# SajayR/TRIAD

Measured on AMD Instinct MI355X. Metric: tri-modal triples/sec (whole node) + loss parity, B=256 at 1/2/4/8 MI355X, higher is better.
Workload: dtype bf16

## Files before the change

### triad_amd/csrc/gemm.hip

```cpp
#include "common.h"

namespace {

constexpr int BM = 128, BN = 128, BK = 64;
constexpr int A_ELEMS = BM * BK, B_ELEMS = BK * BN;

__device__ __forceinline__ int kc_off(int m, int chunk) { return m * BK + ((chunk ^ ((m >> 1) & 7)) << 3); }
__device__ __forceinline__ int nc_off(int k, int col) {
  return k * BN + ((((col >> 3) ^ ((k & 3) << 2))) << 3) + (col & 7);
}

template <bool A_KCONTIG>
__device__ __forceinline__ void stage_a_piece(const bf16* __restrict__ A, long long lda, int m0, int k0, bf16* dst,
                                              int wave, int lane, int u) {
  const int inst = wave * 4 + u;
  if (A_KCONTIG) {
    const int m = inst * 8 + (lane >> 3), cp = lane & 7;
    const int c = cp ^ ((m >> 1) & 7);
    glds16(A + (size_t)(m0 + m) * lda + k0 + c * 8, dst + inst * 512);
  } else {
    const int k = inst * 4 + (lane >> 4), cp = lane & 15;
    const int c = cp ^ ((k & 3) << 2);
    glds16(A + (size_t)(k0 + k) * lda + m0 + c * 8, dst + inst * 512);
  }
}

template <bool A_KCONTIG>
__device__ __forceinline__ void stage_a(const bf16* __restrict__ A, long long lda, int m0, int k0, bf16* dst,
                                        int wave, int lane) {
#pragma unroll
  for (int u = 0; u < 4; ++u) stage_a_piece<A_KCONTIG>(A, lda, m0, k0, dst, wave, lane, u);
}


template <bool B_KCONTIG>
__device__ __forceinline__ void stage_b(const bf16* __restrict__ B, long long ldb, int n0, int k0, bf16* dst,
                                        int wave, int lane) {
  stage_a<B_KCONTIG>(B, ldb, n0, k0, dst, wave, lane);
}

__device__ __forceinline__ bf16x8 frag_tr(const bf16* img, int n0, int s, int lane) {
  const int g = lane >> 4, i = lane & 15, q = i >> 2, p = i & 3, hh = g >> 1;
  const int col = n0 + 16 * (g & 1) + 4 * p;
  const int k0 = 16 * s + 8 * hh + q;
  const s16x4 lo = lds_tr16(img + nc_off(k0, col));
  const s16x4 hi = lds_tr16(img + nc_off(k0 + 4, col));
  bf16x8 r;
  s16x4* rp = (s16x4*)&r;
  rp[0] = lo;
  rp[1] = hi;
  return r;
}

__device__ __forceinline__ float bias_at(const void* bias, int bias_bf16, int n) {
  if (!bias) return 0.f;
  return bias_bf16 ? (float)((const bf16*)bias)[n] : ((const float*)bias)[n];
}

__device__ __forceinline__ void tile_split(int xsplit, int& tile, int& split) {
  const int T = gridDim.x;
  if (xsplit) {
    const int L = blockIdx.y * T + blockIdx.x, c = L % 8, i = L / 8;
    tile = i % T;
    split = c + 8 * (i / T);
    return;
  }
  const int bid = blockIdx.x, q8 = T / 8, r8 = T % 8, x = bid % 8;
  tile = (x < r8 ? x * (q8 + 1) : r8 * (q8 + 1) + (x - r8) * q8) + bid / 8;
  split = blockIdx.y;
}

template <bool A_KCONTIG, bool B_KCONTIG, typename OutT>
__global__ __launch_bounds__(256, 2) void gemm_kernel(const bf16* __restrict__ A, long long lda,
                                                      const bf16* __restrict__ B, long long ldb,
                                                      int M, int N, int Kd, const float* __restrict__ alpha_p,
                                                      OutT* __restrict__ C, long long ldc, int k_per_split,
                                                      long long slab_stride, const void* __restrict__ bias, int bias_bf16, int xsplit) {
  __shared__ __attribute__((aligned(16))) bf16 lds[2 * (A_ELEMS + B_ELEMS)];
  const int lane = threadIdx.x & 63, wave = __builtin_amdgcn_readfirstlane(threadIdx.x >> 6);
  const int wm = wave >> 1, wn = wave & 1;
  const int h = lane >> 5;

  int swz, split;
  tile_split(xsplit, swz, split);
  const int ntn = N / BN;
  const int m0 = (swz / ntn) * BM, n0 = (swz % ntn) * BN;

  f32x16 acc[2][2];
#pragma unroll
  for (int a = 0; a < 2; ++a)
#pragma unroll
    for (int b = 0; b < 2; ++b) acc[a][b] = (f32x16){};

  const int kbeg = split * k_per_split;
  const int nk = min(k_per_split, Kd - kbeg) / BK;
  C += (size_t)split * slab_stride;
  if (nk > 0) {
    stage_a<A_KCONTIG>(A, lda, m0, kbeg, lds, wave, lane);
    stage_b<B_KCONTIG>(B, ldb, n0, kbeg, lds + A_ELEMS, wave, lane);
  }
  for (int kt = 0; kt < nk; ++kt) {
    lds_dma_barrier();
    bf16* const nb = lds + ((kt + 1) & 1) * (A_ELEMS + B_ELEMS);
    const bool pf = kt + 1 < nk;
    if (pf) {
      stage_a<A_KCONTIG>(A, lda, m0, kbeg + (kt + 1) * BK, nb, wave, lane);
      stage_b<B_KCONTIG>(B, ldb, n0, kbeg + (kt + 1) * BK, nb + A_ELEMS, wave, lane);
    }
    const bf16* ai = lds + (kt & 1) * (A_ELEMS + B_ELEMS);
    const bf16* bi = ai + A_ELEMS;
#pragma unroll
    for (int s = 0; s < BK / 16; ++s) {
      bf16x8 af[2], bfr[2];
#pragma unroll
      for (int t = 0; t < 2; ++t) {
        const int mrow = wm * 64 + t * 32;
        if (A_KCONTIG) {
          af[t] = *(const bf16x8*)(ai + kc_off(mrow + (lane & 31), 2 * s + h));
        } else {
          af[t] = frag_tr(ai, mrow, s, lane);
        }
        const int ncol = wn * 64 + t * 32;
        if (B_KCONTIG) {
          bfr[t] = *(const bf16x8*)(bi + kc_off(ncol + (lane & 31), 2 * s + h));
        } else {
          bfr[t] = frag_tr(bi, ncol, s, lane);
        }
      }
#pragma unroll
      for (int a = 0; a < 2; ++a)
#pragma unroll
        for (int b = 0; b < 2; ++b) {
          acc[a][b] = mfma32(af[a], bfr[b], acc[a][b]);
        }
    }
  }

  const float alpha = alpha_p ? *alpha_p : 1.f;
#pragma unroll
  for (int a = 0; a < 2; ++a)
#pragma unroll
    for (int b = 0; b < 2; ++b) {
      const int n = n0 + wn * 64 + b * 32 + (lane & 31);
      const float bn = bias_at(bias, bias_bf16, n);
#pragma unroll
      for (int v = 0; v < 16; ++v) {
        const int m = m0 + wm * 64 + a * 32 + (v & 3) + 8 * (v >> 2) + 4 * h;
        C[(size_t)m * ldc + n] = (OutT)(alpha * acc[a][b][v] + bn);
      }
    }
}

constexpr int GB_M = 256, GB_NB = 3;
constexpr int GB_A = GB_M * BK, GB_ST = GB_A + B_ELEMS;
constexpr int GB_PIECES = 6;


template <bool A_KCONTIG, bool B_KCONTIG>
__device__ __forceinline__ void gb_piece(const bf16* __restrict__ A, long long lda, const bf16* __restrict__ B,
                                         long long ldb, int m0, int n0, int k0, bf16* dst, int wave, int lane,
                                         int u) {
  if (u < 4) {
    const int inst = wave * 4 + u;
    if (A_KCONTIG) {
      const int m = inst * 8 + (lane >> 3), cp = lane & 7;
      const int c = cp ^ ((m >> 1) & 7);
      glds16(A + (size_t)(m0 + m) * lda + k0 + c * 8, dst + inst * 512);
    } else {
      const int half = inst >> 4, ii = inst & 15;
      const int k = ii * 4 + (lane >> 4), cp = lane & 15;
      const int c = cp ^ ((k & 3) << 2);
      glds16(A + (size_t)(k0 + k) * lda + m0 + half * 128 + c * 8, dst + half * (BK * 128) + ii * 512);
    }
  } else {
    const int inst = wave * 2 + (u - 4);
    bf16* bd = dst + GB_A;
    if (B_KCONTIG) {
      const int n = inst * 8 + (lane >> 3), cp = lane & 7;
      const int c = cp ^ ((n >> 1) & 7);
      glds16(B + (size_t)(n0 + n) * ldb + k0 + c * 8, bd + inst * 512);
    } else {
      const int k = inst * 4 + (lane >> 4), cp = lane & 15;
      const int c = cp ^ ((k & 3) << 2);
      glds16(B + (size_t)(k0 + k) * ldb + n0 + c * 8, bd + inst * 512);
    }
  }
}

template <bool A_KCONTIG, bool B_KCONTIG, typename OutT>
__global__ __launch_bounds__(512, 1) void gemm_big_kernel(const bf16* __restrict__ A, long long lda,
                                                          const bf16* __restrict__ B, long long ldb, int M, int N,
                                                          int Kd, const float* __restrict__ alpha_p,
                                                          OutT* __restrict__ C, long long ldc, int k_per_split,
                                                          long long slab_stride, const void* __restrict__ bias, int bias_bf16, int xsplit) {
  __shared__ __attribute__((aligned(16))) bf16 lds[GB_NB * GB_ST];
  const int lane = threadIdx.x & 63, wave = __builtin_amdgcn_readfirstlane(threadIdx.x >> 6);
  const int wm = wave >> 1, wn = wave & 1;
  const int h = lane >> 5;
  int swz, split;
  tile_split(xsplit, swz, split);
  const int ntn = N / BN;
  const int m0 = (swz / ntn) * GB_M, n0 = (swz % ntn) * BN;

  f32x16 acc[2][2];
#pragma unroll
  for (int a = 0; a < 2; ++a)
#pragma unroll
    for (int b = 0; b < 2; ++b) acc[a][b] = (f32x16){};

  const int kbeg = split * k_per_split;
  const int nk = __builtin_amdgcn_readfirstlane(max(0, min(k_per_split, Kd - kbeg)) / BK);
  C += (size_t)split * slab_stride;
#pragma unroll
  for (int p = 0; p < GB_NB - 1; ++p)
    if (p < nk)
#pragma unroll
      for (int u = 0; u < GB_PIECES; ++u)
        gb_piece<A_KCONTIG, B_KCONTIG>(A, lda, B, ldb, m0, n0, kbeg + p * BK, lds + p * GB_ST, wave, lane, u);
  for (int kt = 0; kt < nk; ++kt) {
    if (kt + 1 < nk) TRIAD_VMCNT(GB_PIECES);
    else asm volatile("s_waitcnt vmcnt(0)" ::: "memory");
    __syncthreads();
    const bool pf = kt + GB_NB - 1 < nk;
    bf16* const nb = lds + ((kt + GB_NB - 1) % GB_NB) * GB_ST;
    const int kn = kbeg + (kt + GB_NB - 1) * BK;
    const bf16* ai = lds + (kt % GB_NB) * GB_ST;
    const bf16* bi = ai + GB_A;
#pragma unroll
    for (int s = 0; s < BK / 16; ++s) {
      bf16x8 af[2], bfr[2];
#pragma unroll
      for (int t = 0; t < 2; ++t) {
        const int mrow = wm * 64 + t * 32;
        if (A_KCONTIG) af[t] = *(const bf16x8*)(ai + kc_off(mrow + (lane & 31), 2 * s + h));
        else af[t] = frag_tr(ai + (mrow >> 7) * (BK * 128), mrow & 127, s, lane);
        const int ncol = wn * 64 + t * 32;
        if (B_KCONTIG) bfr[t] = *(const bf16x8*)(bi + kc_off(ncol + (lane & 31), 2 * s + h));
        else bfr[t] = frag_tr(bi, ncol, s, lane);
      }
#pragma unroll
      for (int a = 0; a < 2; ++a)
#pragma unroll
        for (int b = 0; b < 2; ++b) {
          acc[a][b] = mfma32(af[a], bfr[b], acc[a][b]);
          const int mi = s * 4 + a * 2 + b;
          if ((mi & 1) && mi / 2 < GB_PIECES) {
            __builtin_amdgcn_sched_barrier(0);
            if (pf) gb_piece<A_KCONTIG, B_KCONTIG>(A, lda, B, ldb, m0, n0, kn, nb, wave, lane, mi / 2);
            __builtin_amdgcn_sched_barrier(0);
          }
        }
    }
  }

  const float alpha = alpha_p ? *alpha_p : 1.f;
#pragma unroll
  for (int a = 0; a < 2; ++a)
#pragma unroll
    for (int b = 0; b < 2; ++b) {
      const int n = n0 + wn * 64 + b * 32 + (lane & 31);
      const float bn = bias_at(bias, bias_bf16, n);
#pragma unroll
      for (int v = 0; v < 16; ++v) {
        const int m = m0 + wm * 64 + a * 32 + (v & 3) + 8 * (v >> 2) + 4 * h;
        C[(size_t)m * ldc + n] = (OutT)(alpha * acc[a][b][v] + bn);
      }
    }
}

constexpr int GW_M = 256, GW_N = 256;
constexpr int GW_A = GW_M * BK, GW_ST = GW_A + GW_N * BK;

template <bool KCONTIG>
__device__ __forceinline__ void gw_piece_one(const bf16* __restrict__ X, long long ld, int r0, int k0, bf16* img,
                                             int inst, int lane) {
  if (KCONTIG) {
    const int m = inst * 8 + (lane >> 3), cp = lane & 7;
    const int c = cp ^ ((m >> 1) & 7);
    glds16(X + (size_t)(r0 + m) * ld + k0 + c * 8, img + inst * 512);
  } else {
    const int half = inst >> 4, ii = inst & 15;
    const int k = ii * 4 + (lane >> 4), cp = lane & 15;
    const int c = cp ^ ((k & 3) << 2);
    glds16(X + (size_t)(k0 + k) * ld + r0 + half * 128 + c * 8, img + half * (BK * 128) + ii * 512);
  }
}

template <bool KCONTIG>
__device__ __forceinline__ bf16x8 gw_frag(const bf16* img, int row, int s, int lane) {
  if (KCONTIG) return *(const bf16x8*)(img + kc_off(row + (lane & 31), 2 * s + (lane >> 5)));
  return frag_tr(img + (row >> 7) * (BK * 128), row & 127, s, lane);
}

constexpr int GE_PIECES = 8;

template <bool A_KCONTIG, bool B_KCONTIG>
__device__ __forceinline__ void ge_piece(const bf16* __restrict__ A, long long lda, const bf16* __restrict__ B,
                                         long long ldb, int m0, int n0, int k0, bf16* dst, int wave, int lane,
                                         int u) {
  if (u < 4) gw_piece_one<A_KCONTIG>(A, lda, m0, k0, dst, wave * 4 + u, lane);
  else gw_piece_one<B_KCONTIG>(B, ldb, n0, k0, dst + GW_A, wave * 4 + (u - 4), lane);
}

template <bool A_KCONTIG, bool B_KCONTIG, typename OutT>
__global__ __launch_bounds__(512, 1) void gemm_w8_kernel(const bf16* __restrict__ A, long long lda,
                                                         const bf16* __restrict__ B, long long ldb, int M, int N,
                                                         int Kd, const float* __restrict__ alpha_p,
                                                         OutT* __restrict__ C, long long ldc, int k_per_split,
                                                         long long slab_stride, const void* __restrict__ bias, int bias_bf16, int xsplit) {
  __shared__ __attribute__((aligned(16))) bf16 lds[2 * GW_ST];
  const int lane = threadIdx.x & 63, wave = __builtin_amdgcn_readfirstlane(threadIdx.x >> 6);
  const int wm = wave >> 2, wn = wave & 3;
  const int h = lane >> 5;
  int swz, split;
  tile_split(xsplit, swz, split);
  const int ntn = N / GW_N;
  const int m0 = (swz / ntn) * GW_M, n0 = (swz % ntn) * GW_N;

  f32x16 acc[4][2];
#pragma unroll
  for (int a = 0; a < 4; ++a)
#pragma unroll
    for (int b = 0; b < 2; ++b) acc[a][b] = (f32x16){};

  const int kbeg = split * k_per_split;
  const int nk = __builtin_amdgcn_readfirstlane(max(0, min(k_per_split, Kd - kbeg)) / BK);
  C += (size_t)split * slab_stride;
  if (nk > 0)
#pragma unroll
    for (int u = 0; u < GE_PIECES; ++u)
      ge_piece<A_KCONTIG, B_KCONTIG>(A, lda, B, ldb, m0, n0, kbeg, lds, wave, lane, u);
  for (int kt = 0; kt < nk; ++kt) {
    asm volatile("s_waitcnt vmcnt(0)" ::: "memory");
    __syncthreads();
    const bool pf = kt + 1 < nk;
    bf16* const nb = lds + ((kt + 1) & 1) * GW_ST;
    const int kn = kbeg + (kt + 1) * BK;
    const bf16* ai = lds + (kt & 1) * GW_ST;
    const bf16* bi = ai + GW_A;
    bf16x8 af[2][4], bfr[2][2];
#pragma unroll
    for (int t = 0; t < 4; ++t) af[0][t] = gw_frag<A_KCONTIG>(ai, wm * 128 + t * 32, 0, lane);
#pragma unroll
    for (int t = 0; t < 2; ++t) bfr[0][t] = gw_frag<B_KCONTIG>(bi, wn * 64 + t * 32, 0, lane);
#pragma unroll
    for (int s = 0; s < BK / 16; ++s) {
      const int cur = s & 1;
#pragma unroll
      for (int a = 0; a < 4; ++a)
#pragma unroll
        for (int b = 0; b < 2; ++b) {
          acc[a][b] = mfma32(af[cur][a], bfr[cur][b], acc[a][b]);
          const int j = a * 2 + b, mi = s * 8 + j;
          if (s + 1 < BK / 16 && j < 6) {
            __builtin_amdgcn_sched_barrier(0);
            if (j < 4) af[cur ^ 1][j] = gw_frag<A_KCONTIG>(ai, wm * 128 + j * 32, s + 1, lane);
            else bfr[cur ^ 1][j - 4] = gw_frag<B_KCONTIG>(bi, wn * 64 + (j - 4) * 32, s + 1, lane);
            __builtin_amdgcn_sched_barrier(0);
          }
          if (mi % 2 == 1 && mi / 2 < GE_PIECES) {
            __builtin_amdgcn_sched_barrier(0);
            if (pf) ge_piece<A_KCONTIG, B_KCONTIG>(A, lda, B, ldb, m0, n0, kn, nb, wave, lane, mi / 2);
            __builtin_amdgcn_sched_barrier(0);
          }
        }
    }
  }

  const float alpha = alpha_p ? *alpha_p : 1.f;
#pragma unroll
  for (int a = 0; a < 4; ++a)
#pragma unroll
    for (int b = 0; b < 2; ++b) {
      const int n = n0 + wn * 64 + b * 32 + (lane & 31);
      const float bn = bias_at(bias, bias_bf16, n);
#pragma unroll
      for (int v = 0; v < 16; ++v) {
        const int m = m0 + wm * 128 + a * 32 + (v & 3) + 8 * (v >> 2) + 4 * h;
        C[(size_t)m * ldc + n] = (OutT)(alpha * acc[a][b][v] + bn);
      }
    }
}


constexpr int kBigForm = 4;
constexpr int kXcdSplit = 8;
constexpr int kMaxGridY = 65535;


template <bool AK, bool BK_, typename OutT>
int launch(const void* A, long long lda, const void* B, long long ldb, int M, int N, int Kd, const float* alpha,
           void* C, long long ldc, hipStream_t st, int splits = 1, long long slab_stride = 0,
           const void* bias = nullptr, int form = 0, int bias_bf16 = 0) {
  const int xsplit = (form & kXcdSplit) ? 1 : 0;
  form &= ~kXcdSplit;
  if (M <= 0 || N <= 0 || Kd <= 0) return TRIAD_EINVAL;
  if (M % BM || N % BN || Kd % BK || lda % 8 || ldb % 8 || splits < 1) return TRIAD_EINVAL;
  if (xsplit && splits % 8) return TRIAD_EINVAL;
  if (splits > kMaxGridY) return TRIAD_EINVAL;
  if (!A || !B || !C || ldc < N) return TRIAD_EINVAL;
  if ((uintptr_t)A % 16 || (uintptr_t)B % 16) return TRIAD_EINVAL;
  const int kps = ((Kd / BK + splits - 1) / splits) * BK;
  const bool w4_ok = M % GW_M == 0 && N % GW_N == 0;
  const bool w4_auto = AK && BK_ && splits == 1 && M >= 65536 && Kd >= 1024;
  if (form == 0 && w4_ok && w4_auto) form = kBigForm;
  if (w4_ok && (form == 4 || form == 3)) {
    const int nwg = (M / GW_M) * (N / GW_N);
    hipLaunchKernelGGL((gemm_w8_kernel<AK, BK_, OutT>), dim3(nwg, splits), dim3(512), 0, st, (const bf16*)A, lda,
                       (const bf16*)B, ldb, M, N, Kd, alpha, (OutT*)C, ldc, kps, slab_stride, bias, bias_bf16, xsplit);
    TRIAD_CHECK_LAUNCH();
    return TRIAD_OK;
  }
  if (form != 1 && M % GB_M == 0 &&
      (form == 2 || M >= 8192 || Kd / splits >= 32768)) {
    const int nwg = (M / GB_M) * (N / BN);
    hipLaunchKernelGGL((gemm_big_kernel<AK, BK_, OutT>), dim3(nwg, splits), dim3(512), 0, st, (const bf16*)A, lda,
                       (const bf16*)B, ldb, M, N, Kd, alpha, (OutT*)C, ldc, kps, slab_stride, bias, bias_bf16, xsplit);
    TRIAD_CHECK_LAUNCH();
    return TRIAD_OK;
  }
  const int nwg = (M / BM) * (N / BN);
  hipLaunchKernelGGL((gemm_kernel<AK, BK_, OutT>), dim3(nwg, splits), dim3(256), 0, st, (const bf16*)A, lda,
                     (const bf16*)B, ldb, M, N, Kd, alpha, (OutT*)C, ldc, kps, slab_stride, bias, bias_bf16, xsplit);
  TRIAD_CHECK_LAUNCH();
  return TRIAD_OK;
}

}

extern "C" {

int triad_gemm_bf16_form(const void* A, long long lda, int a_kcontig, const void* B, long long ldb, int b_kcontig,
                         int M, int N, int Kd, const float* alpha, void* C, long long ldc, int out_bf16, int form,
                         hipStream_t stream) {
  if (form < 0 || form > 4) return TRIAD_EINVAL;
#define TRIAD_GEMM_CASE(AK, BKC)                                                                  \
  if (!!a_kcontig == AK && !!b_kcontig == BKC)                                                   \
    return out_bf16 ? launch<AK, BKC, bf16>(A, lda, B, ldb, M, N, Kd, alpha, C, ldc, stream, 1, 0, nullptr, form) \
                    : launch<AK, BKC, float>(A, lda, B, ldb, M, N, Kd, alpha, C, ldc, stream, 1, 0, nullptr, form);
  TRIAD_GEMM_CASE(true, true)
  TRIAD_GEMM_CASE(true, false)
  TRIAD_GEMM_CASE(false, true)
  TRIAD_GEMM_CASE(false, false)
#undef TRIAD_GEMM_CASE
  return TRIAD_EINVAL;
}

int triad_gemm_bf16(const void* A, long long lda, int a_kcontig, const void* B, long long ldb, int b_kcontig,
                    int M, int N, int Kd, const float* alpha, void* C, long long ldc, int out_bf16,
                    hipStream_t stream) {
  return triad_gemm_bf16_form(A, lda, a_kcontig, B, ldb, b_kcontig, M, N, Kd, alpha, C, ldc, out_bf16, 0, stream);
}

static int gemm_bias_launch(const void* A, long long lda, int a_kcontig, const void* B, long long ldb, int b_kcontig, int M,
                     int N, int Kd, const void* bias, int bias_bf16, void* C, long long ldc, hipStream_t stream) {
  int form = 1;
  if (M >= 32768 && M % GW_M == 0 && N % GW_N == 0) form = kBigForm;
  else if (M >= 8192 && M % GB_M == 0 && (long long)(M / GB_M) * (N / BN) >= 256) form = 2;
#define TRIAD_GEMM_B(AK, BKC)                                                                     \
  if (!!a_kcontig == AK && !!b_kcontig == BKC)                                                    \
    return launch<AK, BKC, bf16>(A, lda, B, ldb, M, N, Kd, nullptr, C, ldc, stream, 1, 0, bias, form, bias_bf16);
  TRIAD_GEMM_B(true, true)
  TRIAD_GEMM_B(true, false)
  TRIAD_GEMM_B(false, true)
  TRIAD_GEMM_B(false, false)
#undef TRIAD_GEMM_B
  return TRIAD_EINVAL;
}

int triad_gemm_bf16_bias(const void* A, long long lda, int a_kcontig, const void* B, long long ldb, int b_kcontig,
                         int M, int N, int Kd, const float* bias, void* C, long long ldc, hipStream_t stream) {
  return gemm_bias_launch(A, lda, a_kcontig, B, ldb, b_kcontig, M, N, Kd, bias, 0, C, ldc, stream);
}

int triad_gemm_bf16_bias_bf16(const void* A, long long lda, int a_kcontig, const void* B, long long ldb,
                              int b_kcontig, int M, int N, int Kd, const void* bias, void* C, long long ldc,
                              hipStream_t stream) {
  return gemm_bias_launch(A, lda, a_kcontig, B, ldb, b_kcontig, M, N, Kd, bias, 1, C, ldc, stream);
}

int triad_gemm_bf16_splitk_form(const void* A, long long lda, int a_kcontig, const void* B, long long ldb,
                                int b_kcontig, int M, int N, int Kd, int splits, const float* alpha, float* slabs,
                                void* C, int out_bf16, int form, hipStream_t stream) {
  if ((form & ~kXcdSplit) < 0 || (form & ~kXcdSplit) > 4) return TRIAD_EINVAL;
  if (!slabs || !C) return TRIAD_EINVAL;
  const long long slab = (long long)M * N;
  int rc = TRIAD_EINVAL;
#define TRIAD_GEMM_SK(AK, BKC)                                                                  \
  if (!!a_kcontig == AK && !!b_kcontig == BKC)                                                 \
    rc = launch<AK, BKC, float>(A, lda, B, ldb, M, N, Kd, nullptr, slabs, N, stream, splits, slab, nullptr, form);
  TRIAD_GEMM_SK(true, true)
  TRIAD_GEMM_SK(true, false)
  TRIAD_GEMM_SK(false, true)
  TRIAD_GEMM_SK(false, false)
#undef TRIAD_GEMM_SK
  if (rc) return rc;
  return triad_sum_slabs(slabs, splits, slab, alpha, out_bf16, C, stream);
}

int triad_gemm_bf16_splitk(const void* A, long long lda, int a_kcontig, const void* B, long long ldb, int b_kcontig,
                           int M, int N, int Kd, int splits, const float* alpha, float* slabs, void* C,
                           int out_bf16, hipStream_t stream) {
  return triad_gemm_bf16_splitk_form(A, lda, a_kcontig, B, ldb, b_kcontig, M, N, Kd, splits, alpha, slabs, C,
                                     out_bf16, 0, stream);
}

}
```

Before: 1971.

## Restructure wide GEMM mainloop into quadrant-phased pipeline with ping-pong wave scheduling

```diff
diff --git a/triad_amd/csrc/gemm.hip b/triad_amd/csrc/gemm.hip
--- a/triad_amd/csrc/gemm.hip
+++ b/triad_amd/csrc/gemm.hip
@@ -272,34 +272,129 @@
 constexpr int GW_A = GW_M * BK, GW_ST = GW_A + GW_N * BK;
 
 template <bool KCONTIG>
-__device__ __forceinline__ void gw_piece_one(const bf16* __restrict__ X, long long ld, int r0, int k0, bf16* img,
-                                             int inst, int lane) {
-  if (KCONTIG) {
-    const int m = inst * 8 + (lane >> 3), cp = lane & 7;
-    const int c = cp ^ ((m >> 1) & 7);
-    glds16(X + (size_t)(r0 + m) * ld + k0 + c * 8, img + inst * 512);
-  } else {
-    const int half = inst >> 4, ii = inst & 15;
-    const int k = ii * 4 + (lane >> 4), cp = lane & 15;
-    const int c = cp ^ ((k & 3) << 2);
-    glds16(X + (size_t)(k0 + k) * ld + r0 + half * 128 + c * 8, img + half * (BK * 128) + ii * 512);
-  }
-}
-
-template <bool KCONTIG>
 __device__ __forceinline__ bf16x8 gw_frag(const bf16* img, int row, int s, int lane) {
   if (KCONTIG) return *(const bf16x8*)(img + kc_off(row + (lane & 31), 2 * s + (lane >> 5)));
   return frag_tr(img + (row >> 7) * (BK * 128), row & 127, s, lane);
 }
 
-constexpr int GE_PIECES = 8;
-
-template <bool A_KCONTIG, bool B_KCONTIG>
-__device__ __forceinline__ void ge_piece(const bf16* __restrict__ A, long long lda, const bf16* __restrict__ B,
-                                         long long ldb, int m0, int n0, int k0, bf16* dst, int wave, int lane,
-                                         int u) {
-  if (u < 4) gw_piece_one<A_KCONTIG>(A, lda, m0, k0, dst, wave * 4 + u, lane);
-  else gw_piece_one<B_KCONTIG>(B, ldb, n0, k0, dst + GW_A, wave * 4 + (u - 4), lane);
+
+constexpr int GP_LOADS = 2;
+constexpr int GP_FLIGHT = 3;
+enum { GP_STEADY = 0, GP_PENULT = 1, GP_LAST = 2 };
+
+__device__ __forceinline__ void glds16_so(const void* sbase, unsigned voff, void* lds_base) {
+  const unsigned lds = __builtin_amdgcn_readfirstlane((unsigned)(size_t)LDS_PTR(void, lds_base));
+  TRIAD_LDS_DMA_CHECK(lds, 1);
+  unsigned keep;
+  asm volatile(
+      "s_mov_b32 %0, m0\n\t"
+      "s_mov_b32 m0, %3\n\t"
+      "s_nop 2\n\t"
+      "global_load_lds_dwordx4 %1, %2\n\t"
+      "s_mov_b32 m0, %0"
+      : "=&s"(keep)
+      : "v"(voff), "s"(sbase), "s"(lds)
+      : "memory");
+}
+
+template <bool KCONTIG>
+__device__ __forceinline__ unsigned gp_voff(long long ld, int lane, int j) {
+  if (KCONTIG) {
+    const int mr = lane >> 3, c = (lane & 7) ^ (((j * 8 + mr) >> 1) & 7);
+    return (unsigned)((mr * ld + c * 8) * 2);
+  }
+  const int kr = lane >> 4, c = (lane & 15) ^ ((kr & 3) << 2);
+  return (unsigned)((kr * ld + c * 8) * 2);
+}
+
+template <bool KCONTIG>
+__device__ __forceinline__ void gp_piece(const bf16* __restrict__ X, long long ld, int r0, int k0, bf16* img, int inst,
+                                         unsigned voff) {
+  if (KCONTIG) {
+    glds16_so(X + (size_t)(r0 + inst * 8) * ld + k0, voff, img + inst * 512);
+  } else {
+    const int half = inst >> 4, ii = inst & 15;
+    glds16_so(X + (size_t)(k0 + ii * 4) * ld + r0 + half * 128, voff, img + half * (BK * 128) + ii * 512);
+  }
+}
+
+template <bool KCONTIG, bool SUBS>
+__device__ __forceinline__ void gp_half(const bf16* __restrict__ X, long long ld, int r0, int k0, bf16* img, int wave,
+                                        const unsigned (&voff)[2], int hh) {
+#pragma unroll
+  for (int j = 0; j < GP_LOADS; ++j) {
+    const int k = wave * 2 + j;
+    const int inst = SUBS ? (k >> 2) * 8 + hh * 4 + (k & 3) : wave * 4 + hh * 2 + j;
+    gp_piece<KCONTIG>(X, ld, r0, k0, img, inst, voff[j]);
+  }
+}
+
+__device__ __forceinline__ void gp_sync() {
+  __builtin_amdgcn_sched_barrier(0);
+  asm volatile("s_waitcnt lgkmcnt(0)" ::: "memory");
+  __builtin_amdgcn_s_barrier();
+  __builtin_amdgcn_sched_barrier(0);
+}
+
+__device__ __forceinline__ void gp_quadrant(f32x16 (&acc)[4][2], const bf16x8 (&af)[2][4], const bf16x8 (&bf)[4], int ah,
+                                            int b, bool trail = true) {
+  __builtin_amdgcn_s_setprio(1);
+#pragma unroll
+  for (int s = 0; s < BK / 16; ++s)
+#pragma unroll
+    for (int a = 0; a < 2; ++a) acc[2 * ah + a][b] = mfma32(af[a][s], bf[s], acc[2 * ah + a][b]);
+  __builtin_amdgcn_s_setprio(0);
+  __builtin_amdgcn_sched_barrier(0);
+  if (trail) __builtin_amdgcn_s_barrier();
+  __builtin_amdgcn_sched_barrier(0);
+}
+
+template <bool A_KCONTIG, bool B_KCONTIG, int MODE>
+__device__ __forceinline__ void gp_step(const bf16* __restrict__ A, long long lda, const bf16* __restrict__ B,
+                                        long long ldb, int m0, int n0, int kn, bf16* lds, int slot, int wave, int lane,
+                                        int wm, int wn, const unsigned (&va)[2], const unsigned (&vb)[2],
+                                        f32x16 (&acc)[4][2]) {
+  bf16* const cur = lds + slot * GW_ST;
+  bf16* const oth = lds + (slot ^ 1) * GW_ST;
+  const bf16* ai = cur;
+  const bf16* bi = cur + GW_A;
+  bf16x8 af[2][4], bfr[2][4];
+#pragma unroll
+  for (int s = 0; s < 4; ++s) bfr[0][s] = gw_frag<B_KCONTIG>(bi, wn * 64, s, lane);
+#pragma unroll
+  for (int a = 0; a < 2; ++a)
+#pragma unroll
+    for (int s = 0; s < 4; ++s) af[a][s] = gw_frag<A_KCONTIG>(ai, wm * 128 + a * 32, s, lane);
+  if (!B_KCONTIG)
+#pragma unroll
+    for (int s = 0; s < 4; ++s) bfr[1][s] = gw_frag<B_KCONTIG>(bi, wn * 64 + 32, s, lane);
+  __builtin_amdgcn_sched_barrier(0);
+  if (MODE != GP_LAST) gp_half<A_KCONTIG, false>(A, lda, m0, kn, oth, wave, va, 1);
+  gp_sync();
+  gp_quadrant(acc, af, bfr[0], 0, 0);
+  if (B_KCONTIG)
+#pragma unroll
+    for (int s = 0; s < 4; ++s) bfr[1][s] = gw_frag<B_KCONTIG>(bi, wn * 64 + 32, s, lane);
+  __builtin_amdgcn_sched_barrier(0);
+  if (MODE == GP_STEADY) gp_half<B_KCONTIG, B_KCONTIG>(B, ldb, n0, kn + BK, cur + GW_A, wave, vb, 0);
+  gp_sync();
+  gp_quadrant(acc, af, bfr[1], 0, 1);
+#pragma unroll
+  for (int a = 0; a < 2; ++a)
+#pragma unroll
+    for (int s = 0; s < 4; ++s) af[a][s] = gw_frag<A_KCONTIG>(ai, wm * 128 + 64 + a * 32, s, lane);
+  __builtin_amdgcn_sched_barrier(0);
+  if (MODE == GP_STEADY) gp_half<B_KCONTIG, B_KCONTIG>(B, ldb, n0, kn + BK, cur + GW_A, wave, vb, 1);
+  gp_sync();
+  gp_quadrant(acc, af, bfr[1], 1, 1);
+  if (MODE == GP_STEADY) {
+    gp_half<A_KCONTIG, false>(A, lda, m0, kn + BK, cur, wave, va, 0);
+    TRIAD_VMCNT(GP_LOADS * GP_FLIGHT);
+  } else if (MODE == GP_PENULT) {
+    asm volatile("s_waitcnt vmcnt(0)" ::: "memory");
+  }
+  gp_sync();
+  gp_quadrant(acc, af, bfr[0], 1, 0, MODE != GP_LAST || wm == 0);
 }
 
 template <bool A_KCONTIG, bool B_KCONTIG, typename OutT>
@@ -326,45 +421,43 @@
   const int kbeg = split * k_per_split;
   const int nk = __builtin_amdgcn_readfirstlane(max(0, min(k_per_split, Kd - kbeg)) / BK);
   C += (size_t)split * slab_stride;
-  if (nk > 0)
-#pragma unroll
-    for (int u = 0; u < GE_PIECES; ++u)
-      ge_piece<A_KCONTIG, B_KCONTIG>(A, lda, B, ldb, m0, n0, kbeg, lds, wave, lane, u);
-  for (int kt = 0; kt < nk; ++kt) {
-    asm volatile("s_waitcnt vmcnt(0)" ::: "memory");
-    __syncthreads();
-    const bool pf = kt + 1 < nk;
-    bf16* const nb = lds + ((kt + 1) & 1) * GW_ST;
-    const int kn = kbeg + (kt + 1) * BK;
-    const bf16* ai = lds + (kt & 1) * GW_ST;
-    const bf16* bi = ai + GW_A;
-    bf16x8 af[2][4], bfr[2][2];
-#pragma unroll
-    for (int t = 0; t < 4; ++t) af[0][t] = gw_frag<A_KCONTIG>(ai, wm * 128 + t * 32, 0, lane);
-#pragma unroll
-    for (int t = 0; t < 2; ++t) bfr[0][t] = gw_frag<B_KCONTIG>(bi, wn * 64 + t * 32, 0, lane);
-#pragma unroll
-    for (int s = 0; s < BK / 16; ++s) {
-      const int cur = s & 1;
-#pragma unroll
-      for (int a = 0; a < 4; ++a)
-#pragma unroll
-        for (int b = 0; b < 2; ++b) {
-          acc[a][b] = mfma32(af[cur][a], bfr[cur][b], acc[a][b]);
-          const int j = a * 2 + b, mi = s * 8 + j;
-          if (s + 1 < BK / 16 && j < 6) {
-            __builtin_amdgcn_sched_barrier(0);
-            if (j < 4) af[cur ^ 1][j] = gw_frag<A_KCONTIG>(ai, wm * 128 + j * 32, s + 1, lane);
-            else bfr[cur ^ 1][j - 4] = gw_frag<B_KCONTIG>(bi, wn * 64 + (j - 4) * 32, s + 1, lane);
-            __builtin_amdgcn_sched_barrier(0);
-          }
-          if (mi % 2 == 1 && mi / 2 < GE_PIECES) {
-            __builtin_amdgcn_sched_barrier(0);
-            if (pf) ge_piece<A_KCONTIG, B_KCONTIG>(A, lda, B, ldb, m0, n0, kn, nb, wave, lane, mi / 2);
-            __builtin_amdgcn_sched_barrier(0);
-          }
-        }
-    }
+  if (nk > 0) {
+    const unsigned va[2] = {gp_voff<A_KCONTIG>(lda, lane, 0), gp_voff<A_KCONTIG>(lda, lane, 1)};
+    const unsigned vb[2] = {gp_voff<B_KCONTIG>(ldb, lane, 0), gp_voff<B_KCONTIG>(ldb, lane, 1)};
+#pragma unroll
+    for (int hh = 0; hh < 2; ++hh) {
+      gp_half<B_KCONTIG, B_KCONTIG>(B, ldb, n0, kbeg, lds + GW_A, wave, vb, hh);
+      gp_half<A_KCONTIG, false>(A, lda, m0, kbeg, lds, wave, va, hh);
+    }
+    if (nk > 1) {
+      gp_half<B_KCONTIG, B_KCONTIG>(B, ldb, n0, kbeg + BK, lds + GW_ST + GW_A, wave, vb, 0);
+      gp_half<B_KCONTIG, B_KCONTIG>(B, ldb, n0, kbeg + BK, lds + GW_ST + GW_A, wave, vb, 1);
+      gp_half<A_KCONTIG, false>(A, lda, m0, kbeg + BK, lds + GW_ST, wave, va, 0);
+      TRIAD_VMCNT(GP_LOADS * GP_FLIGHT);
+    } else {
+      asm volatile("s_waitcnt vmcnt(0)" ::: "memory");
+    }
+    __builtin_amdgcn_s_barrier();
+    if (wm) __builtin_amdgcn_s_barrier();
+    __builtin_amdgcn_sched_barrier(0);
+#define GP_STEP(slot, MODE, kt)                                                                                \
+  gp_step<A_KCONTIG, B_KCONTIG, MODE>(A, lda, B, ldb, m0, n0, kbeg + ((kt) + 1) * BK, lds, slot, wave, lane, wm, wn, \
+                                      va, vb, acc)
+    int kt = 0;
+    for (; kt + 3 < nk; kt += 2) {
+      GP_STEP(0, GP_STEADY, kt);
+      GP_STEP(1, GP_STEADY, kt + 1);
+    }
+    if (nk - kt == 3) {
+      GP_STEP(0, GP_STEADY, kt);
+      ++kt;
+    }
+    if (nk - kt == 2) {
+      GP_STEP(kt & 1, GP_PENULT, kt);
+      ++kt;
+    }
+    GP_STEP(kt & 1, GP_LAST, kt);
+#undef GP_STEP
   }
 
   const float alpha = alpha_p ? *alpha_p : 1.f;
```

Measured after the change: 2030, median of 6. 3.0% higher.
